# mingfeisun/DeepMimic_mujoco

Hardware: AMD Instinct MI355X
Metric: env-steps/sec (higher is better)
Workload: dtype f64

## Files before the change

### deepmimic_mujoco_amd/csrc/slot_step.h

```cpp
#pragma once

#include "env_step.h"
#include "slot_kernel.h"

namespace dm {

template <class R> struct DofVec { R r[DOF_PASSES]; };

template <class R>
DM_DEV void slot_integrate_pos(SlotShared<R>& s, const DofVec<R>& x0q, int sl, R h) {
  const R q0 = dmw::row_bcast<3>(x0q.r[0]), q1 = dmw::row_bcast<4>(x0q.r[0]), q2 = dmw::row_bcast<5>(x0q.r[0]), q3 = dmw::row_bcast<6>(x0q.r[0]);
  if (sl < 3) s.qpos[sl] = x0q.r[0] + h * s.tau[sl];
  else if (sl == 3) {
    R ax[3] = {s.tau[3], s.tau[4], s.tau[5]}, q[4] = {q0, q1, q2, q3}, qr[4];
    const R angle = h * normalize3(ax);
    if (angle == R(0)) { qr[0] = 1; qr[1] = qr[2] = qr[3] = 0; } else axisangle2quat(qr, ax, angle);
    normalize4(q);
    quat_mul(q, q, qr);
    s.qpos[3] = q[0]; s.qpos[4] = q[1]; s.qpos[5] = q[2]; s.qpos[6] = q[3];
  } else if (sl >= 7) s.qpos[sl] = x0q.r[0] + h * s.tau[sl - 1];
#pragma unroll
  for (int c = 1; c < Q_PASSES; c++) { const int i = sl + SW * c; if (i < NQ) s.qpos[i] = x0q.r[c] + h * s.tau[i - 1]; }
}

template <class R, bool PROF = false, bool CARRY = false, int MAXR = 2 * SW>
DM_DEV void slot_rk4_step(const DevModel<R>& M, SlotShared<R>& s, const SlotTables& tb, int sl, int lane, const LaneTopo& lt, R* xip, int& ovf, long long* prof = 0) {
  const R h = M.timestep;
  const R A[3] = {R(0.5), R(0.5), R(1)};
  const R Bw[4] = {R(1) / 6, R(1) / 3, R(1) / 3, R(1) / 6};
  DofVec<R> x0q, x0v, vprev, aprev, sumv, suma;
#pragma unroll
  for (int c = 0; c < DOF_PASSES; c++) {
    const int i = sl + SW * c;
    x0q.r[c] = i < NQ ? s.qpos[i] : R(0);
    const R v0 = i < NV ? s.qvel[i] : R(0);
    x0v.r[c] = v0; vprev.r[c] = v0; aprev.r[c] = 0; sumv.r[c] = 0; suma.r[c] = 0;
// ... 6 lines not shown
      for (int c = 0; c < DOF_PASSES; c++) { const int d = sl + SW * c; if (d < NV) s.tau[d] = cf * vprev.r[c]; }
      dmw::sync();
      slot_integrate_pos(s, x0q, sl, h);
#pragma unroll
      for (int c = 0; c < DOF_PASSES; c++) {
        const int d = sl + SW * c;
        if (d < NV) { const R vi = x0v.r[c] + h * (cf * aprev.r[c]); vprev.r[c] = vi; s.qvel[d] = vi; }
      }
      dmw::sync();
    }
    typedef decltype(dmw::park(R(0))) ParkedR;
    ParkedR pk[5][DOF_PASSES];
#pragma unroll
    for (int c = 0; c < DOF_PASSES; c++) { pk[0][c] = dmw::park(x0q.r[c]); pk[1][c] = dmw::park(x0v.r[c]); pk[2][c] = dmw::park(vprev.r[c]); pk[3][c] = dmw::park(sumv.r[c]); pk[4][c] = dmw::park(suma.r[c]); }
    slot_forward<R, PROF, CARRY, MAXR>(M, s, tb, sl, lane, lt, xip, ovf, (const DebugOut*)0, prof);
#pragma unroll
    for (int c = 0; c < DOF_PASSES; c++) { x0q.r[c] = dmw::unpark(pk[0][c]); x0v.r[c] = dmw::unpark(pk[1][c]); vprev.r[c] = dmw::unpark(pk[2][c]); sumv.r[c] = dmw::unpark(pk[3][c]); suma.r[c] = dmw::unpark(pk[4][c]); }
#pragma unroll
    for (int c = 0; c < DOF_PASSES; c++) {
      const int d = sl + SW * c;
      if (d < NV) { const R a = s.qd.o.qacc[d]; aprev.r[c] = a; sumv.r[c] += Bw[i] * vprev.r[c]; suma.r[c] += Bw[i] * a; }
    }
  }
#pragma unroll
  for (int c = 0; c < DOF_PASSES; c++) { const int d = sl + SW * c; if (d < NV) s.tau[d] = sumv.r[c]; }
  dmw::sync();
  slot_integrate_pos(s, x0q, sl, h);
#pragma unroll
  for (int c = 0; c < DOF_PASSES; c++) { const int d = sl + SW * c; if (d < NV) { s.qvel[d] = x0v.r[c] + h * suma.r[c]; s.qws[d] = aprev.r[c]; } }
  dmw::sync();
}

template <class R>
DM_DEV void slot_load_env(const DevModel<R>& M, const Batch<R>& B, SlotShared<R>& s, int env, int sl, bool live, const double* action) {
#pragma unroll
  for (int c = 0; c < Q_PASSES; c++) {
    const int i = sl + SW * c;
    if (i < NQ) s.qpos[i] = B.qpos[(size_t)env * NQ + i];
    if (i < NV) { s.qvel[i] = B.qvel[(size_t)env * NV + i]; s.qws[i] = B.qws[(size_t)env * NV + i]; s.act[i] = 0; }
  }
  if (sl == 0) { s.status = 0; s.nefc = 0; s.ncon = 0; s.solver_iter = 0; }
  dmw::sync();
  if (action) {
#pragma unroll
    for (int c = 0; c < HINGE_PASSES; c++) {
      const int u = sl + SW * c;
      if (u < NU) {
        R a = (R)action[(size_t)env * NU + u];
        if (B.action_mode == 1) {
          const int idx = B.frame_idx[env];
          a += R(0.8) * (B.mocap_cfg[(size_t)idx * NQ + 7 + u] - s.qpos[7 + u]);
        } else if (B.action_mode == 2) {
          const int idx = B.frame_idx[env];
          a += M.kp[u + 6] * (B.mocap_cfg[(size_t)idx * NQ + 7 + u] - s.qpos[7 + u]) + M.kd[u + 6] * (B.mocap_vel[(size_t)idx * NV + 6 + u] - s.qvel[6 + u]);
        }
        if (live) B.ctrl[(size_t)env * NU + u] = a;
        const int d = u + 6;
        s.act[d] = M.gear[d] * clampr(a, M.ctrl_lo[d], M.ctrl_hi[d]);
      }
    }
  }
  dmw::sync_mem();
}

template <class R>
DM_DEV void slot_spd_control(const DevModel<R>& M, const Batch<R>& B, SlotShared<R>& s, const SlotTables& tb, int env, int sl, const LaneTopo& lt, bool live,
                             const DofVec<R>& qbar, const DofVec<R>& vbar) {
  const R h = M.timestep;
#pragma unroll
  for (int c = 0; c < DOF_PASSES; c++) { const int d = sl + SW * c; if (d < NV) s.act[d] = 0; }
  dmw::sync();
  R xip[3];
  slot_kinematics(M, s, sl, lt, xip);
  slot_bias(M, s, tb, sl, lt);
  slot_mass_matrix<R, false, true>(M, s, tb, sl, lt, (const DebugOut*)0);
  R pd[DOF_PASSES], kd[DOF_PASSES];
#pragma unroll
  for (int c = 0; c < DOF_PASSES; c++) {
    const int d = sl + SW * c;
    pd[c] = 0; kd[c] = 0;
    if (d >= 6 && d < NV) {
      const R q = s.qpos[d + 1], v = s.qvel[d];
      kd[c] = M.kd[d];
      pd[c] = M.kp[d] * (qbar.r[c] - q - h * v) + kd[c] * (vbar.r[c] - v);
      s.tau[d] += pd[c];
    }
  }
  dmw::sync();
  {
    R x[1][NV];
#pragma unroll
    for (int d = 0; d < NV; d++) x[0][d] = s.tau[d];
    slot_solve_LT<1>(x, s.r2.qLD);
#pragma unroll
    for (int d = 0; d < NV; d++) { x[0][d] *= s.qd.o.dinv[d]; dmw::pin_value(x[0][d]); }
    solve_L(x[0], s.r2.qLD);
    if (sl == 0) {
#pragma unroll
      for (int d = 0; d < NV; d++) s.qd.o.qacc[d] = x[0][d];
    }
  }
  dmw::sync();
#pragma unroll
  for (int c = 0; c < DOF_PASSES; c++) {
    const int d = sl + SW * c;
    if (d >= 6 && d < NV) {
      const R g = M.gear[d];
      const R ct = (pd[c] - h * kd[c] * s.qd.o.qacc[d]) / g;
      if (live) B.ctrl[(size_t)env * NU + (d - 6)] = ct;
      s.act[d] = g * clampr(ct, M.ctrl_lo[d], M.ctrl_hi[d]);
    }
  }
  dmw::sync_mem();
}

template <class R>
DM_DEV void slot_store_state(const Batch<R>& B, SlotShared<R>& s, int env, int sl, bool live) {
  if (!live) return;
#pragma unroll
  for (int c = 0; c < Q_PASSES; c++) {
    const int i = sl + SW * c;
    if (i < NQ) B.qpos[(size_t)env * NQ + i] = s.qpos[i];
    if (i < NV) { B.qvel[(size_t)env * NV + i] = s.qvel[i]; B.qws[(size_t)env * NV + i] = s.qws[i]; }
  }
}

template <class R>
DM_DEV void slot_reset_env(const DevModel<R>& M, const Batch<R>& B, SlotShared<R>& s, int env, int sl, bool doit, int mode, int hard) {
  const int ep = B.episode[env];
  const int genv = B.env_offset + env;
  int idx = (int)(rng_uniform(B.seed, genv, ep, 0) * (double)B.n_frames);
  if (idx >= B.n_frames) idx = B.n_frames - 1;
  if (doit) {
#pragma unroll
    for (int c = 0; c < Q_PASSES; c++) {
      const int i = sl + SW * c;
      if (mode == 0) {
        if (i < NQ) s.qpos[i] = B.mocap_cfg[(size_t)idx * NQ + i];
        if (i < NV) s.qvel[i] = B.mocap_vel[(size_t)idx * NV + i];
      } else if (mode == 1) {
        if (i < NQ) s.qpos[i] = M.qpos0[i] + (R)((rng_uniform(B.seed, genv, ep, 1 + i) * 2.0 - 1.0) * 0.01);
        if (i < NV) s.qvel[i] = (R)((rng_uniform(B.seed, genv, ep, 64 + i) * 2.0 - 1.0) * 0.01);
      } else {
        if (i < NQ) s.qpos[i] = M.qpos0[i];
        if (i < NV) s.qvel[i] = 0;
      }
      if (hard && i < NV) s.qws[i] = 0;
    }
    if (hard && sl == 0) B.time[env] = 0;
  }
  dmw::sync_mem();
  if (doit && sl == 0) {
    B.episode[env] = ep + 1;
    if (mode == 0 || (mode == 1 && hard)) set_frame(B, env, idx); else B.cycle[env] = 0;
  }
}

template <class R>
DM_DEV R slot_imitation_reward(const DevModel<R>& M, const Batch<R>& B, SlotShared<R>& s, int sl, const LaneTopo& lt, const R* ref, R shx, R shy, const R* refv = nullptr) {
  R qloc[4], aloc[3][3], xip[3];
  slot_kinematics(M, s, sl, lt, xip, qloc, aloc);
  const bool v1 = refv != nullptr;
  const R* rv = v1 ? refv : ref;
  const R* P = B.imit_pdev;
  R rq[4] = {s.qpos[3], s.qpos[4], s.qpos[5], s.qpos[6]};
  normalize4(rq);
  R pose = 0, vel = 0, eff = 0, root = 0, mx = 0, my = 0, mz = 0;
  if (sl < 13) {
    const int g = sl - 1;
    const int da = dmw::launder(lt.dofadr), nd = dmw::launder(lt.dofnum);
    const bool isroot = sl == 0, ball = !isroot && nd == 3;
    const R* rquat = ref + (isroot ? 3 : 13 + 4 * g);
    const R ident[4] = {1, 0, 0, 0};
    R q0[4], q1[4];
    for (int k = 0; k < 4; k++) { q0[k] = isroot ? rq[k] : (ball ? qloc[k] : ident[k]); q1[k] = (isroot || ball) ? rquat[k] : ident[k]; }
    const R th = quat_diff_theta(q0, q1);
    R pe = v1 ? fabs(th) : th * th, ve = 0;
    if (isroot) {
      R wv[3];
      const R wloc[3] = {s.qvel[3], s.qvel[4], s.qvel[5]};
      quat_rot(wv, rq, wloc);
      R dv2 = 0, dp2 = 0;
      for (int k = 0; k < 3; k++) { const R a = rv[10 + k] - wv[k]; ve += v1 ? fabs(a) : a * a; const R c = ref[7 + k] - s.qvel[k]; dv2 += c * c; }
      const R p1[3] = {ref[0] + shx, ref[1] + shy, ref[2]};
      for (int k = 0; k < 3; k++) { const R a = s.qpos[k] - p1[k]; dp2 += v1 ? fabs(a) : a * a; }
      root = v1 ? dp2 : dp2 + R(0.1) * pe + R(0.01) * dv2 + R(0.001) * ve;
    } else if (ball) {
      R wl[3] = {0, 0, 0};
      for (int k = 0; k < 3; k++) { const R rate = s.qvel[da + k]; wl[0] += aloc[k][0] * rate; wl[1] += aloc[k][1] * rate; wl[2] += aloc[k][2] * rate; }
      for (int k = 0; k < 3; k++) { const R w = rv[61 + 3 * g + k] - wl[k]; ve += v1 ? fabs(w) : w * w; }
    } else {
      const R a = ref[13 + 4 * g] - s.qpos[da + 1], w = rv[61 + 3 * g] - s.qvel[da];
      pe = v1 ? fabs(a) : a * a; ve = v1 ? fabs(w) + fabs(rv[61 + 3 * g + 1]) + fabs(rv[61 + 3 * g + 2]) : w * w;
    }
    const R wj = v1 ? (isroot ? R(1) : P[g] / P[12]) : P[isroot ? 12 : g];
    pose = wj * pe; vel = v1 ? ve : wj * ve;
  }
  if (sl < 4) {
    const int e = sl, b = (int)P[16 + e];
    const R ex[3] = {1, 0, 0};
    R fwd[3], p[3], rel[3];
    quat_rot(fwd, rq, ex);
    const R hn = sqrt(fwd[0] * fwd[0] + fwd[1] * fwd[1]);
    const R c = hn > R(0) ? fwd[0] / hn : R(1), sn = hn > R(0) ? fwd[1] / hn : R(0);
    mat_vec(p, s.xmat[b], P + 20 + 3 * e);
    for (int k = 0; k < 3; k++) { p[k] += s.xpos[b][k]; rel[k] = p[k] - s.qpos[k]; }
    rel[2] = p[2];
    const R f0[3] = {c * rel[0] + sn * rel[1], -sn * rel[0] + c * rel[1], rel[2]};
    for (int k = 0; k < 3; k++) { const R a = ref[97 + 3 * e + k] - f0[k]; eff += a * a; }
  }
#pragma unroll
  for (int cpass = 0; cpass < DOF_PASSES; cpass++) {
    const int d = sl + SW * cpass;
    if (d < NV) {
      const int b = TOPO.dof_body[d];
      const R* cb = s.r2.i.crb[b];
      const R* cd = s.cdof[d];
      const R qd = s.qvel[d], ms = cb[9];
      R axs[3];
      cross3(axs, cd, cb + 6);
      mx += qd * (ms * cd[3] + axs[0]); my += qd * (ms * cd[4] + axs[1]); mz += qd * (ms * cd[5] + axs[2]);
    }
  }
  pose = dmw::sum16(pose); vel = dmw::sum16(vel); eff = dmw::sum16(eff) / 4; root = dmw::row_bcast<0>(root);
  mx = dmw::sum16(mx) / M.total_mass; my = dmw::sum16(my) / M.total_mass; mz = dmw::sum16(mz) / M.total_mass;
  const R dc[3] = {ref[109] - mx, ref[110] - my, ref[111] - mz};
  const R com = R(0.1) * dot3(dc, dc);
  const R arg = sl == 0 ? R(-2) * pose : sl == 1 ? R(-0.1) * vel : sl == 2 ? (v1 ? R(-5) * root : R(-40) * eff) : sl == 3 ? R(-5) * root : R(-10) * com;
  const R wgt = sl == 0 ? R(0.5) : sl == 1 ? R(0.05) : sl == 2 ? (v1 ? R(0.2) : R(0.15)) : sl == 3 ? R(0.2) : R(0.1);
  R term = 0;
  if (sl < (v1 ? 3 : 5)) term = wgt * exp_once(arg);
  return dmw::sum16(term);
}

template <class R, bool PROF, bool CARRY, int MAXR, bool SPD>
DM_DEV bool slot_env_step_impl(const DevModel<R>& M, const Batch<R>& B, SlotShared<R>& s, SlotTables& tb, int env, int sl, int lane, bool live,
                               const double* action, double* obs, double* reward, unsigned char* done, int n_substeps, int* redo_count, int* redo_list,
                               long long* prof_out = 0, bool kin_carry = false) {
  long long prof[32];
  for (int k = 0; k < 32; k++) prof[k] = 0;
  long long tstart = 0;
  if (PROF) tstart = dmw::clk();
  const LaneTopo lt = lane_topo(sl);
  if constexpr (CARRY) { if (!kin_carry && sl == 0) s.kin_ok() = R(0); }
  DofVec<R> qbar, vbar;
  if constexpr (SPD) {
    slot_load_env(M, B, s, env, sl, live, (const double*)0);
#pragma unroll
    for (int c = 0; c < DOF_PASSES; c++) {
      const int d = sl + SW * c;
      qbar.r[c] = 0; vbar.r[c] = 0;
      if (d >= 6 && d < NV) {
        const int u = d - 6;
        if (action) qbar.r[c] = (R)action[(size_t)env * NU + u];
        if (B.action_mode == 4) {
          const int idx = B.frame_idx[env];
          qbar.r[c] += B.mocap_cfg[(size_t)idx * NQ + 7 + u];
          vbar.r[c] = B.mocap_vel[(size_t)idx * NV + 6 + u];
        }
      }
    }
  } else
  slot_load_env(M, B, s, env, sl, live, action);
  R xip[3];
  int why = 0;
  for (int k = 0; k < n_substeps; k++) {
    if constexpr (SPD) slot_spd_control(M, B, s, tb, env, sl, lt, live, qbar, vbar);
    slot_rk4_step<R, PROF, CARRY, MAXR>(M, s, tb, sl, lane, lt, xip, why, prof);
  }
  const bool ovf = dmw::row_ballot(why != 0, lane) != 0u;
  if (dmw::ballot(ovf) != 0ull) {
    unsigned bits = 0;
    for (int r = 0; r < 5; r++) if (dmw::row_ballot(((why >> r) & 1) != 0, lane) != 0u) bits |= 1u << r;
    if (ovf && live && sl == 0) {
      if (redo_count) { const int k = dmw::global_counter_next(redo_count); redo_list[k] = env; }
      for (int r = 0; r < 5; r++) if ((bits >> r) & 1u) dmw::global_counter_next(B.redo_why + 1 + r);
    }
  }
  live = live && !ovf;
  const R mz = sl < NB - 1 ? M.body_mass[sl + 1] * xip[2] : R(0);
  const R z = dmw::sum16(mz) / M.total_mass;
  bool dn = (z < R(0.7)) || (z > R(2.0));
  if (live) {
    if (B.diag != 0) {
      if (sl < NB - 1) for (int k = 0; k < 3; k++) B.xipos[(size_t)env * NB * 3 + 3 * (sl + 1) + k] = xip[k];
      if (sl < 3) B.xipos[(size_t)env * NB * 3 + sl] = 0;
      const int nc = s.ncon;
      for (int k = sl; k < MAXEFC * 2; k += SW) {
        const int c = k >> 1;
        int gid = -1;
        if (c < nc && c < SLOT_MAXCON) { const auto& rec = M.pair_rec[s.r1.rw.coni[c] & 0xff]; gid = (k & 1) ? rec.g2 : rec.g1; }
        B.cong[(size_t)env * MAXEFC * 2 + k] = gid;
      }
    }
    if (sl == 0) { B.comz[env] = z; B.ncon[env] = s.ncon; B.nefc[env] = s.nefc; B.status[env] = s.status; B.solver_iter[env] = s.solver_iter; if constexpr (!CARRY) order_ticket(B, env, s.nefc, s.solver_iter); }
  }
  R rew = 1;
  if (B.reward_mode == REW_V3_CONFIG) {
    const int idx = B.frame_idx[env];
    R err = 0;
    for (int i = 7; i < NQ; i++) err += fabs(s.qpos[i] - B.mocap_cfg[(size_t)idx * NQ + i]);
    rew = exp_once(-err);
    dmw::sync_mem();
    if (live && sl == 0) B.frame_idx[env] = (idx + 1) % B.n_frames;
  } else if (B.reward_mode == REW_V2_POSE) {
    const int idx = B.frame_idx[env] + 1;
    const int im = (idx + B.frame_init[env]) % B.n_frames;
    R err = 0, acs = 0;
    for (int i = 3; i < NQ; i++) err += fabs(s.qpos[i] - B.mocap_cfg[(size_t)im * NQ + i]);
    for (int u = 0; u < NU; u++) { const R c = B.ctrl[(size_t)env * NU + u]; acs += c * c; }
    rew = exp_once(R(-2) * err) - R(0.1) * acs;
    dmw::sync_mem();
    if (live && sl == 0) B.frame_idx[env] = idx;
  } else if (B.reward_mode == REW_IMITATION) {
    int k = B.frame_idx[env] + 1, cyc = B.cycle[env];
    bool ended = false;
    if (k >= B.n_frames) { if (B.imit_params[15] != R(0)) { k = 0; cyc += 1; } else { k = B.n_frames - 1; ended = true; } }
    rew = slot_imitation_reward(M, B, s, sl, lt, B.imit_table + (size_t)k * IMIT_FEAT, cyc * B.imit_params[13], cyc * B.imit_params[14]);
    dn = dn || ended;
    dmw::sync_mem();
    if (live && sl == 0) { B.frame_idx[env] = k; B.cycle[env] = cyc; }
  } else if (B.reward_mode == REW_V1_QUAT) {
    const int idx = B.frame_idx[env] + 1;
    int upd = (int)floor(B.mocap_dt / (M.timestep * n_substeps));
    if (upd < 1) upd = 1;
    const int k = (idx / upd + B.frame_init[env]) % B.n_frames, kv = k + 1 < B.n_frames ? k + 1 : B.n_frames - 1;
    const R robs = slot_imitation_reward(M, B, s, sl, lt, B.imit_table + (size_t)k * IMIT_FEAT, R(0), R(0), B.imit_table + (size_t)kv * IMIT_FEAT);
    R acs = 0;
    for (int u = 0; u < NU; u++) { const R c = B.ctrl[(size_t)env * NU + u]; acs += c * c; }
    rew = (idx % upd == 0 ? robs : R(0)) - R(0.1) * acs;
    dmw::sync_mem();
    if (live && sl == 0) B.frame_idx[env] = idx;
  }
  if (live && sl == 0) { B.time[env] += M.timestep * n_substeps; reward[env] = rew; done[env] = dn ? 1 : 0; if (B.kin) B.kin_ok[env] = 0; }
  if (B.autoreset) {
    dmw::sync_mem();
    slot_reset_env(M, B, s, env, sl, dn && live, B.autoreset == 1 ? 0 : 1, 1);
  }
  if constexpr (CARRY) { if (sl == 0) s.kin_ok() = (B.reward_mode >= REW_IMITATION && !ovf && !(dn && B.autoreset != 0)) ? R(1) : R(0); }
  if (live) {
#pragma unroll
    for (int c = 0; c < (NOBS + SW - 1) / SW; c++) {
      const int o = sl + SW * c;
      if (o < 28) obs[(size_t)env * NOBS + o] = s.qpos[7 + o];
      else if (o < NOBS) obs[(size_t)env * NOBS + o] = s.qvel[6 + (o - 28)];
    }
  }
  slot_store_state(B, s, env, sl, live);
  if (PROF && lane == 0) {
    prof[5] = dmw::clk() - tstart;
    for (int k = 0; k < 32; k++) prof_out[k] = prof[k];
  }
  return live;
}
template <class R, bool PROF = false, bool CARRY = false, int MAXR = 2 * SW>
DM_DEV bool slot_env_step(const DevModel<R>& M, const Batch<R>& B, SlotShared<R>& s, SlotTables& tb, int env, int sl, int lane, bool live,
                          const double* action, double* obs, double* reward, unsigned char* done, int n_substeps, int* redo_count, int* redo_list,
                          long long* prof_out = 0, bool kin_carry = false) {
  if (B.action_mode >= 3) return slot_env_step_impl<R, PROF, CARRY, MAXR, true>(M, B, s, tb, env, sl, lane, live, action, obs, reward, done, n_substeps, redo_count, redo_list, prof_out, kin_carry);
  return slot_env_step_impl<R, PROF, CARRY, MAXR, false>(M, B, s, tb, env, sl, lane, live, action, obs, reward, done, n_substeps, redo_count, redo_list, prof_out, kin_carry);
}

#ifdef DM_STATIC_CALLS
#define DM_CALL_SLOT_PARAM , int* call_slot
#define DM_CALL_SLOT_TOUCH(v) (*call_slot = (v))
#define DM_CALL_SLOT_ARG , &call_slot_mem
#define DM_CALL_SLOT_DECL int call_slot_mem = 0; asm volatile("" :: "v"(&call_slot_mem) : "memory")
#define DM_CALL_SLOT_USE asm volatile("" :: "v"(call_slot_mem))
#else
#define DM_CALL_SLOT_PARAM
#define DM_CALL_SLOT_TOUCH(v) ((void)0)
#define DM_CALL_SLOT_ARG
#define DM_CALL_SLOT_DECL ((void)0)
#define DM_CALL_SLOT_USE ((void)0)
#endif
template <class R> union SlotOrOne {
  SlotShared<R> sh[SLOTS];
  struct { Shared<R> s; StepScratch<R> x; } one;
};
template <class R, int NR>
DM_DEV_CALL64 void restep_one_env(const DevModel<R>* M, const Batch<R>* B, Shared<R>* s, StepScratch<R>* x, int env, int lane, const double* action, double* obs,
                                    double* reward, unsigned char* done, int n_substeps DM_CALL_SLOT_PARAM) {
  DM_CALL_SLOT_TOUCH(0);
  using dmw::uniform_ptr; using dmw::in_lds; using dmw::in_global; using dmw::in_constant;
  const Batch<R> Bv = *in_constant(B);
  env_step_impl<R, NR, false, false>(*in_constant(M), global_members(Bv), *in_lds(uniform_ptr(s)), *in_lds(uniform_ptr(x)), dmw::uniform(env), lane, in_global(uniform_ptr(action)),
                  in_global(uniform_ptr(obs)), in_global(uniform_ptr(reward)), in_global(uniform_ptr(done)), dmw::uniform(n_substeps));
}
template <class R, int MAXR>
DM_DEV_CALL64 int slot_env_step_call(const DevModel<R>* M, const Batch<R>* B, SlotShared<R>* s, SlotTables* tb, int env, int sl, int lane, bool live,
                                     const double* action, double* obs, double* reward, unsigned char* done, int n_substeps, int kin_carry DM_CALL_SLOT_PARAM) {
  using dmw::uniform_ptr; using dmw::in_lds; using dmw::in_global; using dmw::in_constant;
  const Batch<R> Bv = *in_constant(B);
  SlotShared<R>& sr = *in_lds(s);
  DM_CALL_SLOT_TOUCH(env);
  const bool stored = slot_env_step_impl<R, false, true, MAXR, false>(*in_constant(M), global_members(Bv), sr, *in_lds(uniform_ptr(tb)), env, sl, lane, live, in_global(uniform_ptr(action)),
                                                          in_global(uniform_ptr(obs)), in_global(uniform_ptr(reward)), in_global(uniform_ptr(done)), dmw::uniform(n_substeps), (int*)0, (int*)0,
                                                          (long long*)0, dmw::uniform(kin_carry) != 0);
  return (stored ? 1 : 0) | (sr.nefc << 8);
}
#ifdef DM_ROLLOUT_PROF
template <class R, int MAXR>
DM_DEV_CALL64 int slot_env_step_call_prof(const DevModel<R>* M, const Batch<R>* B, SlotShared<R>* s, SlotTables* tb, int env, int sl, int lane, bool live,
                                          const double* action, double* obs, double* reward, unsigned char* done, int n_substeps, long long* prof_out, int kin_carry DM_CALL_SLOT_PARAM) {
  DM_CALL_SLOT_TOUCH(env);
  using dmw::uniform_ptr; using dmw::in_lds; using dmw::in_global; using dmw::in_constant;
  const Batch<R> Bv = *in_constant(B);
  SlotShared<R>& sr = *in_lds(s);
  const bool stored = slot_env_step_impl<R, true, true, MAXR, false>(*in_constant(M), global_members(Bv), sr, *in_lds(uniform_ptr(tb)), env, sl, lane, live, in_global(uniform_ptr(action)),
                                                         in_global(uniform_ptr(obs)), in_global(uniform_ptr(reward)), in_global(uniform_ptr(done)), dmw::uniform(n_substeps), (int*)0, (int*)0,
                                                         in_global(uniform_ptr(prof_out)), dmw::uniform(kin_carry) != 0);
  return (stored ? 1 : 0) | (sr.nefc << 8);
}
#endif
struct StepRow { const double* action; double* obs; double* reward; unsigned char* done; };
#ifndef DM_EXT_MARGIN
#define DM_EXT_MARGIN 9
#endif
constexpr int EXT_MARGIN = DM_EXT_MARGIN;
template <class R, int NR, class POLICY>
DM_DEV void slot_rollout(const DevModel<R>& M_in, const Batch<R>& B, SlotShared<R>* sh, SlotTables& tb, Shared<R>& one_s, StepScratch<R>& one_x,
                         int env, int lane, bool live, const StepRow* rows, int n_substeps, int T, POLICY&& policy, long long* prof_acc = 0, bool policy_clobbers_kin = false) {
  const int slot = lane >> 4, sl = lane & 15;
  int carry = 0;
  int last_rows = B.nefc[env];
  DM_CALL_SLOT_DECL;
  for (int t = 0; t < T; t++) {
    const DevModel<R>& M = *dmw::launder_uniform_ptr(&M_in);
    const StepRow row = rows[t];
    const double* a_t = row.action;
    double* o_t = row.obs;
    double* r_t = row.reward;
    unsigned char* d_t = row.done;
    const bool heavy = rows_max(last_rows) > 2 * SW - EXT_MARGIN;
    int ret;
#ifdef DM_ROLLOUT_PROF
    if (prof_acc) {
      ret = heavy ? slot_env_step_call_prof<R, SLOT_MAXROWS>(&M, &B, &sh[slot], &tb, env, sl, lane, live, a_t, o_t, r_t, d_t, n_substeps, prof_acc + 32, carry DM_CALL_SLOT_ARG)
                  : slot_env_step_call_prof<R, 2 * SW>(&M, &B, &sh[slot], &tb, env, sl, lane, live, a_t, o_t, r_t, d_t, n_substeps, prof_acc + 32, carry DM_CALL_SLOT_ARG);
      if (lane == 0) { for (int k = 0; k < 31; k++) prof_acc[k] += prof_acc[32 + k]; if (heavy) prof_acc[28] += 1; }
    } else
// ... 34 lines not shown
```

### deepmimic_mujoco_amd/csrc/wave.h

```cpp
#pragma once

#if defined(DM_WAVE_TESTBENCH)
#include "wave_testbench.h"
#else
#include <hip/hip_runtime.h>

#define DM_DEV __device__ __forceinline__
#define DM_DEV_NOINLINE __device__ __noinline__
#ifndef DM_NO_STATIC_CALLS
#define DM_STATIC_CALLS 1
#define DM_DEV_CALL64 static __device__ __noinline__
#else
#define DM_DEV_CALL64 __device__ __noinline__
#endif
#define DM_CONSTANT __device__ constexpr

namespace dmw {
DM_DEV int lane() { return (int)(threadIdx.x & 63u); }
DM_DEV void sync() { __builtin_amdgcn_fence(__ATOMIC_SEQ_CST, "wavefront"); __builtin_amdgcn_wave_barrier(); }
DM_DEV void sync_mem() { __syncthreads(); }
DM_DEV unsigned long long ballot(bool p) { return __ballot(p); }
DM_DEV int shfl_i(int v, int src) { return __shfl(v, src, 64); }
DM_DEV double shfl(double v, int src) { return __shfl(v, src, 64); }
DM_DEV float shfl(float v, int src) { return __shfl(v, src, 64); }
// ... 41 lines not shown
  c = __builtin_amdgcn_mfma_f64_16x16x4f64(a, b, c, 0, 0, 0);
  d[0] = c[0]; d[1] = c[1]; d[2] = c[2]; d[3] = c[3];
}
DM_DEV void mfma_16x16x4(float a, float b, float (&d)[4]) {
  typedef float v4f __attribute__((ext_vector_type(4)));
  v4f c = {d[0], d[1], d[2], d[3]};
  c = __builtin_amdgcn_mfma_f32_16x16x4f32(a, b, c, 0, 0, 0);
  d[0] = c[0]; d[1] = c[1]; d[2] = c[2]; d[3] = c[3];
}
DM_DEV int mfma_row(int lane_id, int v, double) { return (lane_id >> 4) + 4 * v; }
DM_DEV int mfma_row(int lane_id, int v, float) { return 4 * (lane_id >> 4) + v; }
DM_DEV double max_raw(double a, double b) { double r; asm("v_max_f64 %0, %1, %2" : "=v"(r) : "v"(a), "v"(b)); return r; }
DM_DEV float max_raw(float a, float b) { float r; asm("v_max_f32 %0, %1, %2" : "=v"(r) : "v"(a), "v"(b)); return r; }
DM_DEV long long clk() { return (long long)__builtin_readcyclecounter(); }
DM_DEV void sched_fence() { __builtin_amdgcn_sched_barrier(0); }
DM_DEV int pin_zero() { int z = 0; asm volatile("" : "+s"(z)); return z; }
DM_DEV void pin_value(double& v) { asm volatile("" : "+v"(v)); }
DM_DEV void pin_value(float& v) { asm volatile("" : "+v"(v)); }
DM_DEV int launder(int v) { asm volatile("" : "+v"(v)); return v; }
DM_DEV int launder_slot_lane(int v) { asm volatile("" : "+v"(v)); __builtin_assume(v >= 0 && v < 16); return v; }
DM_DEV unsigned long long launder(unsigned long long v) { asm volatile("" : "+v"(v)); return v; }
DM_DEV int launder_uniform(int v) { asm volatile("" : "+s"(v)); return v; }
template <class T> DM_DEV T* uniform_ptr(T* p) {
  const unsigned long long v = (unsigned long long)p;
  const unsigned lo = __builtin_amdgcn_readfirstlane((unsigned)v), hi = __builtin_amdgcn_readfirstlane((unsigned)(v >> 32));
  return (T*)(((unsigned long long)hi << 32) | lo);
}
template <class T> DM_DEV T* in_lds(T* p) {
#if defined(__HIP_DEVICE_COMPILE__)
  __builtin_assume(__builtin_amdgcn_is_shared((const void*)p));
#endif
  return p;
}
template <class T> DM_DEV T* in_global(T* p) {
  __attribute__((address_space(1))) T* g = (__attribute__((address_space(1))) T*)uniform_ptr(p);
  asm volatile("" : "+s"(g));
  return (T*)g;
}
template <class T> DM_DEV const T* in_constant(const T* p) {
  __attribute__((address_space(4))) const T* g = (__attribute__((address_space(4))) const T*)uniform_ptr(p);
  asm volatile("" : "+s"(g));
  return (const T*)g;
}
template <class T> DM_DEV T* launder_uniform_ptr(T* p) { asm volatile("" : "+s"(p)); return p; }
DM_DEV void reload_fence() { asm volatile("" ::: "memory"); }
DM_DEV void lds_sub(bool pred, double* p, double v) { if (pred) __hip_atomic_fetch_add(p, -v, __ATOMIC_RELAXED, __HIP_MEMORY_SCOPE_WORKGROUP); }
DM_DEV void lds_sub(bool pred, float* p, float v) { if (pred) __hip_atomic_fetch_add(p, -v, __ATOMIC_RELAXED, __HIP_MEMORY_SCOPE_WORKGROUP); }
template <int I> DM_DEV double row_bcast(double v) {
  long long x = __double_as_longlong(v);
  x = __builtin_amdgcn_update_dpp(0ll, x, 0x150 + I, 0xf, 0xf, true);
  return __longlong_as_double(x);
}
template <int I> DM_DEV float row_bcast(float v) { return __int_as_float(__builtin_amdgcn_update_dpp(0, __float_as_int(v), 0x150 + I, 0xf, 0xf, true)); }
template <int I> DM_DEV int row_bcast_i(int v) { return __builtin_amdgcn_update_dpp(0, v, 0x150 + I, 0xf, 0xf, true); }
template <int I> DM_DEV void row_fmac(double& acc, double x, double y) {
  asm volatile("s_nop 1\n\tv_fmac_f64_dpp %0, %1, %2 row_newbcast:%3 row_mask:0xf bank_mask:0xf" : "+v"(acc) : "v"(x), "v"(y), "n"(I));
}
template <int I> DM_DEV void row_fmac(float& acc, float x, float y) { acc += row_bcast<I>(x) * y; }
template <int I> DM_DEV void row_fmac_old(double& acc, double x, double y) {
  asm volatile("s_nop 1\n\tv_fmac_f64_dpp %0, %1, %2 row_newbcast:%3 row_mask:0xf bank_mask:0xf" : "+v"(acc) : "v"(x), "v"(y), "n"(I));
}
template <int I> DM_DEV void row_fmac_old(float& acc, float x, float y) { acc += row_bcast<I>(x) * y; }
#define DM_FMAC_DPP(acc, x, y) "v_fmac_f64_dpp " acc ", " x ", " y " row_newbcast:%18 row_mask:0xf bank_mask:0xf\n\t"
template <int I> DM_DEV void row_fmac8(double& acc0, double& acc1, const double* x, const double* y) {
  asm volatile("s_nop 1\n\t" DM_FMAC_DPP("%0", "%2", "%10") DM_FMAC_DPP("%1", "%3", "%11") DM_FMAC_DPP("%0", "%4", "%12") DM_FMAC_DPP("%1", "%5", "%13")
               DM_FMAC_DPP("%0", "%6", "%14") DM_FMAC_DPP("%1", "%7", "%15") DM_FMAC_DPP("%0", "%8", "%16") DM_FMAC_DPP("%1", "%9", "%17")
// ... 115 lines not shown
```

Baseline: 20.54 million.

## Batch global loads ahead of LDS stores and defer per-env epilogue writes

```diff
diff --git a/deepmimic_mujoco_amd/csrc/slot_step.h b/deepmimic_mujoco_amd/csrc/slot_step.h
--- a/deepmimic_mujoco_amd/csrc/slot_step.h
+++ b/deepmimic_mujoco_amd/csrc/slot_step.h
@@ -2,6 +2,12 @@
 
 #include "env_step.h"
 #include "slot_kernel.h"
+
+#if defined(DM_WAVE_TESTBENCH)
+#define DM_ARRIVED(v) ((void)0)
+#else
+#define DM_ARRIVED(v) asm volatile("" :: "v"(v))
+#endif
 
 namespace dm {
 
@@ -74,35 +80,73 @@
 }
 
 template <class R>
-DM_DEV void slot_load_env(const DevModel<R>& M, const Batch<R>& B, SlotShared<R>& s, int env, int sl, bool live, const double* action) {
+DM_DEV void slot_load_env(const DevModel<R>& M, const Batch<R>& B, SlotShared<R>& s, int env, int sl, bool live, const double* action, LaneTopo& lt, bool clear_kin) {
+  lt = lane_topo(sl);
+  env = dmw::launder(env); sl = dmw::launder_slot_lane(sl);
+  R q[Q_PASSES], v[Q_PASSES], w[Q_PASSES];
+#pragma unroll
+  for (int c = 0; c < Q_PASSES; c++) {
+    const int i = sl + SW * c, iq = i < NQ ? i : NQ - 1, iv = i < NV ? i : NV - 1;
+    q[c] = B.qpos[(size_t)env * NQ + iq];
+    v[c] = B.qvel[(size_t)env * NV + iv];
+    w[c] = B.qws[(size_t)env * NV + iv];
+  }
+  const bool track = action && (B.action_mode == 1 || B.action_mode == 2);
+  R a[HINGE_PASSES], gr[HINGE_PASSES], lo[HINGE_PASSES], hi[HINGE_PASSES];
+  int idx = 0;
+  if (action) {
+#pragma unroll
+    for (int c = 0; c < HINGE_PASSES; c++) {
+      const int u = sl + SW * c, uc = u < NU ? u : NU - 1, d = uc + 6;
+      a[c] = (R)action[(size_t)env * NU + uc];
+      gr[c] = M.gear[d]; lo[c] = M.ctrl_lo[d]; hi[c] = M.ctrl_hi[d];
+    }
+    if (track) idx = B.frame_idx[env];
+  }
+  dmw::sched_fence();
+#if !defined(DM_WAVE_TESTBENCH)
+  asm volatile("" : "+v"(lt.parent), "+v"(lt.dofadr), "+v"(lt.dofnum), "+v"(lt.depth), "+v"(lt.subtree), "+v"(lt.tri));
+#endif
+  if (clear_kin && sl == 0) s.kin_ok() = R(0);
 #pragma unroll
   for (int c = 0; c < Q_PASSES; c++) {
     const int i = sl + SW * c;
-    if (i < NQ) s.qpos[i] = B.qpos[(size_t)env * NQ + i];
-    if (i < NV) { s.qvel[i] = B.qvel[(size_t)env * NV + i]; s.qws[i] = B.qws[(size_t)env * NV + i]; s.act[i] = 0; }
+    if (i < NQ) s.qpos[i] = q[c];
+    if (i < NV) { s.qvel[i] = v[c]; s.qws[i] = w[c]; s.act[i] = 0; }
   }
   if (sl == 0) { s.status = 0; s.nefc = 0; s.ncon = 0; s.solver_iter = 0; }
   dmw::sync();
   if (action) {
+    if (track) {
+      R mq[HINGE_PASSES], mv[HINGE_PASSES], kp[HINGE_PASSES], kd[HINGE_PASSES];
+      const bool pd = B.action_mode == 2;
+#pragma unroll
+      for (int c = 0; c < HINGE_PASSES; c++) {
+        const int u = sl + SW * c, uc = u < NU ? u : NU - 1;
+        mq[c] = B.mocap_cfg[(size_t)idx * NQ + 7 + uc];
+        mv[c] = 0; kp[c] = 0; kd[c] = 0;
+        if (pd) { mv[c] = B.mocap_vel[(size_t)idx * NV + 6 + uc]; kp[c] = M.kp[uc + 6]; kd[c] = M.kd[uc + 6]; }
+      }
+      dmw::sched_fence();
+#pragma unroll
+      for (int c = 0; c < HINGE_PASSES; c++) {
+        const int u = sl + SW * c;
+        if (u < NU) {
+          if (pd) a[c] += kp[c] * (mq[c] - s.qpos[7 + u]) + kd[c] * (mv[c] - s.qvel[6 + u]);
+          else a[c] += R(0.8) * (mq[c] - s.qpos[7 + u]);
+        }
+      }
+    }
 #pragma unroll
     for (int c = 0; c < HINGE_PASSES; c++) {
       const int u = sl + SW * c;
       if (u < NU) {
-        R a = (R)action[(size_t)env * NU + u];
-        if (B.action_mode == 1) {
-          const int idx = B.frame_idx[env];
-          a += R(0.8) * (B.mocap_cfg[(size_t)idx * NQ + 7 + u] - s.qpos[7 + u]);
-        } else if (B.action_mode == 2) {
-          const int idx = B.frame_idx[env];
-          a += M.kp[u + 6] * (B.mocap_cfg[(size_t)idx * NQ + 7 + u] - s.qpos[7 + u]) + M.kd[u + 6] * (B.mocap_vel[(size_t)idx * NV + 6 + u] - s.qvel[6 + u]);
-        }
-        if (live) B.ctrl[(size_t)env * NU + u] = a;
-        const int d = u + 6;
-        s.act[d] = M.gear[d] * clampr(a, M.ctrl_lo[d], M.ctrl_hi[d]);
-      }
-    }
-  }
-  dmw::sync_mem();
+        if (live) B.ctrl[(size_t)env * NU + u] = a[c];
+        s.act[u + 6] = gr[c] * clampr(a[c], lo[c], hi[c]);
+      }
+    }
+  }
+  dmw::sync();
 }
 
 template <class R>
@@ -157,29 +201,32 @@
 }
 
 template <class R>
-DM_DEV void slot_store_state(const Batch<R>& B, SlotShared<R>& s, int env, int sl, bool live) {
-  if (!live) return;
-#pragma unroll
-  for (int c = 0; c < Q_PASSES; c++) {
-    const int i = sl + SW * c;
-    if (i < NQ) B.qpos[(size_t)env * NQ + i] = s.qpos[i];
-    if (i < NV) { B.qvel[(size_t)env * NV + i] = s.qvel[i]; B.qws[(size_t)env * NV + i] = s.qws[i]; }
-  }
-}
-
-template <class R>
 DM_DEV void slot_reset_env(const DevModel<R>& M, const Batch<R>& B, SlotShared<R>& s, int env, int sl, bool doit, int mode, int hard) {
+  if (dmw::ballot(doit) == 0ull) return;
+  DM_MARK("slot_reset");
+  sl = dmw::launder_slot_lane(sl);
+  dmw::sync_mem();
   const int ep = B.episode[env];
   const int genv = B.env_offset + env;
   int idx = (int)(rng_uniform(B.seed, genv, ep, 0) * (double)B.n_frames);
   if (idx >= B.n_frames) idx = B.n_frames - 1;
+  R mq[Q_PASSES], mv[Q_PASSES];
+#pragma unroll
+  for (int c = 0; c < Q_PASSES; c++) {
+    const int i = sl + SW * c, iq = i < NQ ? i : NQ - 1, iv = i < NV ? i : NV - 1;
+    mq[c] = 0; mv[c] = 0;
+    if (mode == 0) { mq[c] = B.mocap_cfg[(size_t)idx * NQ + iq]; mv[c] = B.mocap_vel[(size_t)idx * NV + iv]; }
+  }
+  dmw::sched_fence();
+#pragma unroll
+  for (int c = 0; c < Q_PASSES; c++) { DM_ARRIVED(mq[c]); DM_ARRIVED(mv[c]); }
   if (doit) {
 #pragma unroll
     for (int c = 0; c < Q_PASSES; c++) {
       const int i = sl + SW * c;
       if (mode == 0) {
-        if (i < NQ) s.qpos[i] = B.mocap_cfg[(size_t)idx * NQ + i];
-        if (i < NV) s.qvel[i] = B.mocap_vel[(size_t)idx * NV + i];
+        if (i < NQ) s.qpos[i] = mq[c];
+        if (i < NV) s.qvel[i] = mv[c];
       } else if (mode == 1) {
         if (i < NQ) s.qpos[i] = M.qpos0[i] + (R)((rng_uniform(B.seed, genv, ep, 1 + i) * 2.0 - 1.0) * 0.01);
         if (i < NV) s.qvel[i] = (R)((rng_uniform(B.seed, genv, ep, 64 + i) * 2.0 - 1.0) * 0.01);
@@ -198,13 +245,37 @@
   }
 }
 
+template <class R> struct ImitOperands { R fq[4], fr[3], fp[3], fv[3], fc[3], fe[3], po[3], pb, pw, p12; int db[DOF_PASSES]; };
 template <class R>
-DM_DEV R slot_imitation_reward(const DevModel<R>& M, const Batch<R>& B, SlotShared<R>& s, int sl, const LaneTopo& lt, const R* ref, R shx, R shy, const R* refv = nullptr) {
+DM_DEV void slot_imitation_operands(const Batch<R>& B, int sl, int k, int kv, ImitOperands<R>& o) {
+  const R* ref = B.imit_table + (size_t)k * IMIT_FEAT;
+  const R* rv = B.imit_table + (size_t)(kv >= 0 ? kv : k) * IMIT_FEAT;
+  const R* P = B.imit_pdev;
+  const bool isroot = sl == 0;
+  const int g = sl - 1, gc = g < 0 ? 0 : (g > 11 ? 11 : g), e = sl & 3;
+  const int qa = isroot ? 3 : 13 + 4 * gc, ra = isroot ? 10 : 61 + 3 * gc;
+#pragma unroll
+  for (int j = 0; j < 4; j++) o.fq[j] = ref[qa + j];
+#pragma unroll
+  for (int j = 0; j < 3; j++) { o.fr[j] = rv[ra + j]; o.fp[j] = ref[j]; o.fv[j] = ref[7 + j]; o.fc[j] = ref[109 + j]; o.fe[j] = ref[97 + 3 * e + j]; o.po[j] = P[20 + 3 * e + j]; }
+  o.pb = P[16 + e]; o.pw = P[isroot ? 12 : gc]; o.p12 = P[12];
+#pragma unroll
+  for (int c = 0; c < DOF_PASSES; c++) { const int d = sl + SW * c; o.db[c] = TOPO.dof_body[d < NV ? d : NV - 1]; }
+}
+template <class R>
+DM_DEV R slot_imitation_reward(const DevModel<R>& M, const Batch<R>& B, SlotShared<R>& s, int sl, const LaneTopo& lt, int k, R shx, R shy, int kv = -1) {
   R qloc[4], aloc[3][3], xip[3];
+  ImitOperands<R> o;
+#ifdef DM_REWARD_OPERANDS_EARLY
+  slot_imitation_operands(B, sl, k, kv, o);
+#endif
   slot_kinematics(M, s, sl, lt, xip, qloc, aloc);
-  const bool v1 = refv != nullptr;
-  const R* rv = v1 ? refv : ref;
-  const R* P = B.imit_pdev;
+  DM_MARK("slot_reward_terms");
+#ifndef DM_REWARD_OPERANDS_EARLY
+  slot_imitation_operands(B, sl, k, kv, o);
+#endif
+  dmw::sched_fence();
+  const bool v1 = kv >= 0;
   R rq[4] = {s.qpos[3], s.qpos[4], s.qpos[5], s.qpos[6]};
   normalize4(rq);
   R pose = 0, vel = 0, eff = 0, root = 0, mx = 0, my = 0, mz = 0;
@@ -212,10 +283,9 @@
     const int g = sl - 1;
     const int da = dmw::launder(lt.dofadr), nd = dmw::launder(lt.dofnum);
     const bool isroot = sl == 0, ball = !isroot && nd == 3;
-    const R* rquat = ref + (isroot ? 3 : 13 + 4 * g);
     const R ident[4] = {1, 0, 0, 0};
     R q0[4], q1[4];
-    for (int k = 0; k < 4; k++) { q0[k] = isroot ? rq[k] : (ball ? qloc[k] : ident[k]); q1[k] = (isroot || ball) ? rquat[k] : ident[k]; }
+    for (int k = 0; k < 4; k++) { q0[k] = isroot ? rq[k] : (ball ? qloc[k] : ident[k]); q1[k] = (isroot || ball) ? o.fq[k] : ident[k]; }
     const R th = quat_diff_theta(q0, q1);
     R pe = v1 ? fabs(th) : th * th, ve = 0;
     if (isroot) {
@@ -223,39 +293,39 @@
       const R wloc[3] = {s.qvel[3], s.qvel[4], s.qvel[5]};
       quat_rot(wv, rq, wloc);
       R dv2 = 0, dp2 = 0;
-      for (int k = 0; k < 3; k++) { const R a = rv[10 + k] - wv[k]; ve += v1 ? fabs(a) : a * a; const R c = ref[7 + k] - s.qvel[k]; dv2 += c * c; }
-      const R p1[3] = {ref[0] + shx, ref[1] + shy, ref[2]};
+      for (int k = 0; k < 3; k++) { const R a = o.fr[k] - wv[k]; ve += v1 ? fabs(a) : a * a; const R c = o.fv[k] - s.qvel[k]; dv2 += c * c; }
+      const R p1[3] = {o.fp[0] + shx, o.fp[1] + shy, o.fp[2]};
       for (int k = 0; k < 3; k++) { const R a = s.qpos[k] - p1[k]; dp2 += v1 ? fabs(a) : a * a; }
       root = v1 ? dp2 : dp2 + R(0.1) * pe + R(0.01) * dv2 + R(0.001) * ve;
     } else if (ball) {
       R wl[3] = {0, 0, 0};
       for (int k = 0; k < 3; k++) { const R rate = s.qvel[da + k]; wl[0] += aloc[k][0] * rate; wl[1] += aloc[k][1] * rate; wl[2] += aloc[k][2] * rate; }
-      for (int k = 0; k < 3; k++) { const R w = rv[61 + 3 * g + k] - wl[k]; ve += v1 ? fabs(w) : w * w; }
+      for (int k = 0; k < 3; k++) { const R w = o.fr[k] - wl[k]; ve += v1 ? fabs(w) : w * w; }
     } else {
-      const R a = ref[13 + 4 * g] - s.qpos[da + 1], w = rv[61 + 3 * g] - s.qvel[da];
-      pe = v1 ? fabs(a) : a * a; ve = v1 ? fabs(w) + fabs(rv[61 + 3 * g + 1]) + fabs(rv[61 + 3 * g + 2]) : w * w;
-    }
-    const R wj = v1 ? (isroot ? R(1) : P[g] / P[12]) : P[isroot ? 12 : g];
+      const R a = o.fq[0] - s.qpos[da + 1], w = o.fr[0] - s.qvel[da];
+      pe = v1 ? fabs(a) : a * a; ve = v1 ? fabs(w) + fabs(o.fr[1]) + fabs(o.fr[2]) : w * w;
+    }
+    const R wj = v1 ? (isroot ? R(1) : o.pw / o.p12) : o.pw;
     pose = wj * pe; vel = v1 ? ve : wj * ve;
   }
   if (sl < 4) {
-    const int e = sl, b = (int)P[16 + e];
+    const int b = (int)o.pb;
     const R ex[3] = {1, 0, 0};
     R fwd[3], p[3], rel[3];
     quat_rot(fwd, rq, ex);
     const R hn = sqrt(fwd[0] * fwd[0] + fwd[1] * fwd[1]);
     const R c = hn > R(0) ? fwd[0] / hn : R(1), sn = hn > R(0) ? fwd[1] / hn : R(0);
-    mat_vec(p, s.xmat[b], P + 20 + 3 * e);
+    mat_vec(p, s.xmat[b], o.po);
     for (int k = 0; k < 3; k++) { p[k] += s.xpos[b][k]; rel[k] = p[k] - s.qpos[k]; }
     rel[2] = p[2];
     const R f0[3] = {c * rel[0] + sn * rel[1], -sn * rel[0] + c * rel[1], rel[2]};
-    for (int k = 0; k < 3; k++) { const R a = ref[97 + 3 * e + k] - f0[k]; eff += a * a; }
+    for (int k = 0; k < 3; k++) { const R a = o.fe[k] - f0[k]; eff += a * a; }
   }
 #pragma unroll
   for (int cpass = 0; cpass < DOF_PASSES; cpass++) {
     const int d = sl + SW * cpass;
     if (d < NV) {
-      const int b = TOPO.dof_body[d];
+      const int b = o.db[cpass];
       const R* cb = s.r2.i.crb[b];
       const R* cd = s.cdof[d];
       const R qd = s.qvel[d], ms = cb[9];
@@ -266,7 +336,7 @@
   }
   pose = dmw::sum16(pose); vel = dmw::sum16(vel); eff = dmw::sum16(eff) / 4; root = dmw::row_bcast<0>(root);
   mx = dmw::sum16(mx) / M.total_mass; my = dmw::sum16(my) / M.total_mass; mz = dmw::sum16(mz) / M.total_mass;
-  const R dc[3] = {ref[109] - mx, ref[110] - my, ref[111] - mz};
+  const R dc[3] = {o.fc[0] - mx, o.fc[1] - my, o.fc[2] - mz};
   const R com = R(0.1) * dot3(dc, dc);
   const R arg = sl == 0 ? R(-2) * pose : sl == 1 ? R(-0.1) * vel : sl == 2 ? (v1 ? R(-5) * root : R(-40) * eff) : sl == 3 ? R(-5) * root : R(-10) * com;
   const R wgt = sl == 0 ? R(0.5) : sl == 1 ? R(0.05) : sl == 2 ? (v1 ? R(0.2) : R(0.15)) : sl == 3 ? R(0.2) : R(0.1);
@@ -281,13 +351,13 @@
                                long long* prof_out = 0, bool kin_carry = false) {
   long long prof[32];
   for (int k = 0; k < 32; k++) prof[k] = 0;
-  long long tstart = 0;
+  long long tstart = 0, tepi = 0;
   if (PROF) tstart = dmw::clk();
-  const LaneTopo lt = lane_topo(sl);
-  if constexpr (CARRY) { if (!kin_carry && sl == 0) s.kin_ok() = R(0); }
+  DM_MARK("slot_entry");
+  LaneTopo lt;
   DofVec<R> qbar, vbar;
   if constexpr (SPD) {
-    slot_load_env(M, B, s, env, sl, live, (const double*)0);
+    slot_load_env(M, B, s, env, sl, live, (const double*)0, lt, CARRY && !kin_carry);
 #pragma unroll
     for (int c = 0; c < DOF_PASSES; c++) {
       const int d = sl + SW * c;
@@ -303,13 +373,24 @@
       }
     }
   } else
-  slot_load_env(M, B, s, env, sl, live, action);
+  slot_load_env(M, B, s, env, sl, live, action, lt, CARRY && !kin_carry);
+  if (PROF) prof[29] = dmw::clk() - tstart;
   R xip[3];
   int why = 0;
   for (int k = 0; k < n_substeps; k++) {
     if constexpr (SPD) slot_spd_control(M, B, s, tb, env, sl, lt, live, qbar, vbar);
     slot_rk4_step<R, PROF, CARRY, MAXR>(M, s, tb, sl, lane, lt, xip, why, prof);
   }
+  DM_MARK("slot_rk_end");
+  if (PROF) tepi = dmw::clk();
+  env = dmw::launder(env);
+  const int rmode = B.reward_mode;
+  int cur = 0, cyc = 0, finit = 0;
+  if (rmode != REW_ALIVE) cur = B.frame_idx[env];
+  if (rmode == REW_IMITATION) cyc = B.cycle[env];
+  if (rmode == REW_V2_POSE || rmode == REW_V1_QUAT) finit = B.frame_init[env];
+  R tm = B.time[env];
+  const R bmass = M.body_mass[sl < NB - 1 ? sl + 1 : 0];
   const bool ovf = dmw::row_ballot(why != 0, lane) != 0u;
   if (dmw::ballot(ovf) != 0ull) {
     unsigned bits = 0;
@@ -320,77 +401,97 @@
     }
   }
   live = live && !ovf;
-  const R mz = sl < NB - 1 ? M.body_mass[sl + 1] * xip[2] : R(0);
+  const R mz = sl < NB - 1 ? bmass * xip[2] : R(0);
   const R z = dmw::sum16(mz) / M.total_mass;
   bool dn = (z < R(0.7)) || (z > R(2.0));
-  if (live) {
-    if (B.diag != 0) {
-      if (sl < NB - 1) for (int k = 0; k < 3; k++) B.xipos[(size_t)env * NB * 3 + 3 * (sl + 1) + k] = xip[k];
-      if (sl < 3) B.xipos[(size_t)env * NB * 3 + sl] = 0;
-      const int nc = s.ncon;
-      for (int k = sl; k < MAXEFC * 2; k += SW) {
-        const int c = k >> 1;
-        int gid = -1;
-        if (c < nc && c < SLOT_MAXCON) { const auto& rec = M.pair_rec[s.r1.rw.coni[c] & 0xff]; gid = (k & 1) ? rec.g2 : rec.g1; }
-        B.cong[(size_t)env * MAXEFC * 2 + k] = gid;
-      }
-    }
-    if (sl == 0) { B.comz[env] = z; B.ncon[env] = s.ncon; B.nefc[env] = s.nefc; B.status[env] = s.status; B.solver_iter[env] = s.solver_iter; if constexpr (!CARRY) order_ticket(B, env, s.nefc, s.solver_iter); }
-  }
   R rew = 1;
-  if (B.reward_mode == REW_V3_CONFIG) {
-    const int idx = B.frame_idx[env];
+  int cur_new = cur;
+  if (rmode == REW_V3_CONFIG) {
+    const int idx = cur;
     R err = 0;
     for (int i = 7; i < NQ; i++) err += fabs(s.qpos[i] - B.mocap_cfg[(size_t)idx * NQ + i]);
     rew = exp_once(-err);
-    dmw::sync_mem();
-    if (live && sl == 0) B.frame_idx[env] = (idx + 1) % B.n_frames;
-  } else if (B.reward_mode == REW_V2_POSE) {
-    const int idx = B.frame_idx[env] + 1;
-    const int im = (idx + B.frame_init[env]) % B.n_frames;
+    cur_new = (idx + 1) % B.n_frames;
+  } else if (rmode == REW_V2_POSE) {
+    const int idx = cur + 1;
+    const int im = (idx + finit) % B.n_frames;
     R err = 0, acs = 0;
     for (int i = 3; i < NQ; i++) err += fabs(s.qpos[i] - B.mocap_cfg[(size_t)im * NQ + i]);
     for (int u = 0; u < NU; u++) { const R c = B.ctrl[(size_t)env * NU + u]; acs += c * c; }
     rew = exp_once(R(-2) * err) - R(0.1) * acs;
-    dmw::sync_mem();
-    if (live && sl == 0) B.frame_idx[env] = idx;
-  } else if (B.reward_mode == REW_IMITATION) {
-    int k = B.frame_idx[env] + 1, cyc = B.cycle[env];
+    cur_new = idx;
+  } else if (rmode == REW_IMITATION) {
+    int k = cur + 1;
     bool ended = false;
     if (k >= B.n_frames) { if (B.imit_params[15] != R(0)) { k = 0; cyc += 1; } else { k = B.n_frames - 1; ended = true; } }
-    rew = slot_imitation_reward(M, B, s, sl, lt, B.imit_table + (size_t)k * IMIT_FEAT, cyc * B.imit_params[13], cyc * B.imit_params[14]);
+    rew = slot_imitation_reward(M, B, s, sl, lt, k, cyc * B.imit_params[13], cyc * B.imit_params[14]);
     dn = dn || ended;
-    dmw::sync_mem();
-    if (live && sl == 0) { B.frame_idx[env] = k; B.cycle[env] = cyc; }
-  } else if (B.reward_mode == REW_V1_QUAT) {
-    const int idx = B.frame_idx[env] + 1;
+    cur_new = k;
+  } else if (rmode == REW_V1_QUAT) {
+    const int idx = cur + 1;
     int upd = (int)floor(B.mocap_dt / (M.timestep * n_substeps));
     if (upd < 1) upd = 1;
-    const int k = (idx / upd + B.frame_init[env]) % B.n_frames, kv = k + 1 < B.n_frames ? k + 1 : B.n_frames - 1;
-    const R robs = slot_imitation_reward(M, B, s, sl, lt, B.imit_table + (size_t)k * IMIT_FEAT, R(0), R(0), B.imit_table + (size_t)kv * IMIT_FEAT);
+    const int k = (idx / upd + finit) % B.n_frames, kv = k + 1 < B.n_frames ? k + 1 : B.n_frames - 1;
+    const R robs = slot_imitation_reward(M, B, s, sl, lt, k, R(0), R(0), kv);
     R acs = 0;
     for (int u = 0; u < NU; u++) { const R c = B.ctrl[(size_t)env * NU + u]; acs += c * c; }
     rew = (idx % upd == 0 ? robs : R(0)) - R(0.1) * acs;
-    dmw::sync_mem();
-    if (live && sl == 0) B.frame_idx[env] = idx;
-  }
-  if (live && sl == 0) { B.time[env] += M.timestep * n_substeps; reward[env] = rew; done[env] = dn ? 1 : 0; if (B.kin) B.kin_ok[env] = 0; }
-  if (B.autoreset) {
-    dmw::sync_mem();
-    slot_reset_env(M, B, s, env, sl, dn && live, B.autoreset == 1 ? 0 : 1, 1);
-  }
-  if constexpr (CARRY) { if (sl == 0) s.kin_ok() = (B.reward_mode >= REW_IMITATION && !ovf && !(dn && B.autoreset != 0)) ? R(1) : R(0); }
+    cur_new = idx;
+  }
+  DM_ARRIVED(tm); DM_ARRIVED(cur); DM_ARRIVED(cyc); DM_ARRIVED(finit);
+  DM_MARK("slot_stores");
+  dmw::sync();
   if (live) {
-#pragma unroll
-    for (int c = 0; c < (NOBS + SW - 1) / SW; c++) {
-      const int o = sl + SW * c;
-      if (o < 28) obs[(size_t)env * NOBS + o] = s.qpos[7 + o];
-      else if (o < NOBS) obs[(size_t)env * NOBS + o] = s.qvel[6 + (o - 28)];
-    }
-  }
-  slot_store_state(B, s, env, sl, live);
+    const int nc = s.ncon, ne = s.nefc, st = s.status, it = s.solver_iter;
+    if (B.diag != 0) {
+      int gid[(MAXEFC * 2 + SW - 1) / SW];
+#pragma unroll
+      for (int j = 0; j < (MAXEFC * 2 + SW - 1) / SW; j++) {
+        const int k = sl + SW * j, c = k >> 1;
+        gid[j] = -1;
+        if (k < MAXEFC * 2 && c < nc && c < SLOT_MAXCON) { const auto& rec = M.pair_rec[s.r1.rw.coni[c] & 0xff]; gid[j] = (k & 1) ? rec.g2 : rec.g1; }
+      }
+      dmw::sched_fence();
+      if (sl < NB - 1) for (int k = 0; k < 3; k++) B.xipos[(size_t)env * NB * 3 + 3 * (sl + 1) + k] = xip[k];
+      if (sl < 3) B.xipos[(size_t)env * NB * 3 + sl] = 0;
+#pragma unroll
+      for (int j = 0; j < (MAXEFC * 2 + SW - 1) / SW; j++) { const int k = sl + SW * j; if (k < MAXEFC * 2) B.cong[(size_t)env * MAXEFC * 2 + k] = gid[j]; }
+    }
+    if (sl == 0) {
+      B.comz[env] = z; B.ncon[env] = nc; B.nefc[env] = ne; B.status[env] = st; B.solver_iter[env] = it;
+      if constexpr (!CARRY) order_ticket(B, env, ne, it);
+      if (rmode != REW_ALIVE) B.frame_idx[env] = cur_new;
+      if (rmode == REW_IMITATION) B.cycle[env] = cyc;
+      tm += M.timestep * n_substeps;
+      B.time[env] = tm; reward[env] = rew; done[env] = dn ? 1 : 0; if (B.kin) B.kin_ok[env] = 0;
+    }
+  }
+  if (B.autoreset) slot_reset_env(M, B, s, env, sl, dn && live, B.autoreset == 1 ? 0 : 1, 1);
+  if constexpr (CARRY) { if (sl == 0) s.kin_ok() = (rmode >= REW_IMITATION && !ovf && !(dn && B.autoreset != 0)) ? R(1) : R(0); }
+  DM_MARK("slot_stores");
+  if (live) {
+    sl = dmw::launder_slot_lane(sl);
+    R ov[(NOBS + SW - 1) / SW], sq[Q_PASSES], sv[Q_PASSES], sw[Q_PASSES];
+#pragma unroll
+    for (int c = 0; c < (NOBS + SW - 1) / SW; c++) { const int o = sl + SW * c; ov[c] = o < 28 ? s.qpos[7 + o] : s.qvel[6 + ((o < NOBS ? o : NOBS - 1) - 28)]; }
+#pragma unroll
+    for (int c = 0; c < Q_PASSES; c++) {
+      const int i = sl + SW * c, iq = i < NQ ? i : NQ - 1, iv = i < NV ? i : NV - 1;
+      sq[c] = s.qpos[iq]; sv[c] = s.qvel[iv]; sw[c] = s.qws[iv];
+    }
+    dmw::sched_fence();
+#pragma unroll
+    for (int c = 0; c < (NOBS + SW - 1) / SW; c++) { const int o = sl + SW * c; if (o < NOBS) obs[(size_t)env * NOBS + o] = ov[c]; }
+#pragma unroll
+    for (int c = 0; c < Q_PASSES; c++) {
+      const int i = sl + SW * c;
+      if (i < NQ) B.qpos[(size_t)env * NQ + i] = sq[c];
+      if (i < NV) { B.qvel[(size_t)env * NV + i] = sv[c]; B.qws[(size_t)env * NV + i] = sw[c]; }
+    }
+  }
   if (PROF && lane == 0) {
     prof[5] = dmw::clk() - tstart;
+    prof[30] = dmw::clk() - tepi;
     for (int k = 0; k < 32; k++) prof_out[k] = prof[k];
   }
   return live;
@@ -434,7 +535,11 @@
                                      const double* action, double* obs, double* reward, unsigned char* done, int n_substeps, int kin_carry DM_CALL_SLOT_PARAM) {
   using dmw::uniform_ptr; using dmw::in_lds; using dmw::in_global; using dmw::in_constant;
   const Batch<R> Bv = *in_constant(B);
+#if defined(DM_WAVE_TESTBENCH)
   SlotShared<R>& sr = *in_lds(s);
+#else
+  SlotShared<R>& sr = *dmw::in_lds_lane(s);
+#endif
   DM_CALL_SLOT_TOUCH(env);
   const bool stored = slot_env_step_impl<R, false, true, MAXR, false>(*in_constant(M), global_members(Bv), sr, *in_lds(uniform_ptr(tb)), env, sl, lane, live, in_global(uniform_ptr(action)),
                                                           in_global(uniform_ptr(obs)), in_global(uniform_ptr(reward)), in_global(uniform_ptr(done)), dmw::uniform(n_substeps), (int*)0, (int*)0,
@@ -448,7 +553,11 @@
   DM_CALL_SLOT_TOUCH(env);
   using dmw::uniform_ptr; using dmw::in_lds; using dmw::in_global; using dmw::in_constant;
   const Batch<R> Bv = *in_constant(B);
+#if defined(DM_WAVE_TESTBENCH)
   SlotShared<R>& sr = *in_lds(s);
+#else
+  SlotShared<R>& sr = *dmw::in_lds_lane(s);
+#endif
   const bool stored = slot_env_step_impl<R, true, true, MAXR, false>(*in_constant(M), global_members(Bv), sr, *in_lds(uniform_ptr(tb)), env, sl, lane, live, in_global(uniform_ptr(action)),
                                                          in_global(uniform_ptr(obs)), in_global(uniform_ptr(reward)), in_global(uniform_ptr(done)), dmw::uniform(n_substeps), (int*)0, (int*)0,
                                                          in_global(uniform_ptr(prof_out)), dmw::uniform(kin_carry) != 0);
diff --git a/deepmimic_mujoco_amd/csrc/wave.h b/deepmimic_mujoco_amd/csrc/wave.h
--- a/deepmimic_mujoco_amd/csrc/wave.h
+++ b/deepmimic_mujoco_amd/csrc/wave.h
@@ -97,6 +97,11 @@
 #endif
   return p;
 }
+template <class T> DM_DEV T* in_lds_lane(T* p) {
+  __attribute__((address_space(3))) T* l = (__attribute__((address_space(3))) T*)p;
+  asm volatile("" : "+v"(l));
+  return (T*)l;
+}
 template <class T> DM_DEV T* in_global(T* p) {
   __attribute__((address_space(1))) T* g = (__attribute__((address_space(1))) T*)uniform_ptr(p);
   asm volatile("" : "+s"(g));
```

After: 20.62 million, median of 2. Within noise of the previous version (+0.4%).
